# shivangchopra11/MedMoE

Measured on AMD Instinct MI355X. Metric: image-text pairs/sec at global batch 1024, higher is better.
Workload: dtype bf16; 1 GPU; cfg2: ViT-B/16 + 12-layer text tower (frozen), 8 experts top-2, 224x224x3 + 77 tokens, fwd+bwd+clip+Adam; global_batch=1024, per_gpu_batch=1024, parallelism=dp1

## Files before the change

### medmoe_amd/csrc/gemm.hip

```cpp
#include "common.h"
#include "det_plan.h"
#include <utility>

#define BM 128
#define BN 128
#define BK 64

__device__ __attribute__((aligned(256))) bf16_t g_zero_page[2048];

struct GemmNTArgs {
  const bf16_t* A; const bf16_t* B; void* C;
  const float* bias; const bf16_t* residual; bf16_t* aux;
  const int* a_rowmap; const int* c_rowmap; const int4* tiles; const int* tile_count;
  long long strideB; long long strideBias;
  int M, N, K, lda, ldb, ldc, ldr, ldaux;
  int n_tiles_n, max_tiles_m;
  float alpha; int epi; int out_f32; int col_perm;
  const int* m_dev;
};

static int g_use_nt256 = 1, g_use_nt512 = 1, g_use_tn512 = 1, g_tn_rows = 1024, g_nt_max_grid = 256, g_use_scores512 = 1, g_use_nt4w = 1, g_use_tn4w = 1, g_tn_min_rows = 2048, g_tn_rows4w = 0, g_scores_skip_epi = 0;
#ifdef NT_EXPERIMENT
__device__ int g_nt_dbg_skip = 0;
#define NT_X(...) __VA_ARGS__
#else
#define NT_X(...)
#endif
#ifdef NT_TIMING
__device__ unsigned long long g_nt_timing[8 * 8];
#define NT_T(...) __VA_ARGS__
__device__ __forceinline__ long long nt_clk() {
  __builtin_amdgcn_sched_barrier(0); const long long c = clock64(); __builtin_amdgcn_sched_barrier(0); return c;
}
#else
#define NT_T(...)
#endif
extern int g_attn_resident;
extern int g_sa_rows;
extern int g_attn_rt13;
static int g_last_nt_kernel = -1;
extern "C" int medmoe_last_gemm_nt_kernel() { return g_last_nt_kernel; }
extern int g_ln_one_row;
int g_use_nt_direct = 1;
extern "C" int medmoe_set_option(int key, int value) {
  if (key == 16) { g_ln_one_row = value; return MM_OK; }
  if (key == 17) { g_use_nt_direct = value; return MM_OK; }
  if (key == 1) { g_use_nt256 = value; return MM_OK; }
  if (key == 2) { g_use_nt512 = value; return MM_OK; }
  if (key == 3) { g_use_tn512 = value; return MM_OK; }
  if (key == 4 && value >= 256) { g_tn_rows = value; return MM_OK; }
  if (key == 5 && value >= 1 && value <= 256) { g_nt_max_grid = value; return MM_OK; }
  if (key == 6) { g_use_scores512 = value; return MM_OK; }
  if (key == 7) { g_use_nt4w = value; return MM_OK; }
  if (key == 8) { g_use_tn4w = value; return MM_OK; }
  if (key == 9 && value >= 64) { g_tn_min_rows = value; return MM_OK; }
  if (key == 12) { g_scores_skip_epi = value; return MM_OK; }
  if (key == 15 && (value == 0 || value == 448 || value == 512)) { g_attn_rt13 = value; return MM_OK; }
  if (key == 13 && value >= 0) { g_sa_rows = value; return MM_OK; }
  if (key == 11) { g_attn_resident = value; return MM_OK; }
  if (key == 10 && value >= 0) { g_tn_rows4w = value; return MM_OK; }
  return MM_ERR_ARG;
}

enum { EPI_NONE = 0, EPI_GELU = 1, EPI_RELU = 2, EPI_MUL_DGELU = 3, EPI_MUL_DRELU = 4, EPI_GELU_DAUX = 5, EPI_MUL_AUX = 6 };

struct ParkedTile {
  uint4 c[8];
  int m_base, n_base, n_items, next;
};

typedef unsigned u32x4e_t __attribute__((ext_vector_type(4)));
template <bool PARK, int TM0 = 0, int TMS = 4, int TN0 = 0, int TNS = 4, bool LDSX = false>
__device__ __forceinline__ int nt_epilogue(const GemmNTArgs& p, f32x4_t (&acc)[TMS][TNS], int m_base, int m_end,
                                           int n_base, int group, int frag_row, int frag_q, ParkedTile* park, unsigned lds_x = 0u) {
  int n_stores = 0;
  const int pg = ((frag_q & 1) << 1) | (frag_q >> 1);
  long long mc[4];
  bool mok[4];
#pragma unroll
  for (int tm = 0; tm < 4; ++tm) {
    const int m = m_base + tm * 16 + frag_row;
    mok[tm] = m < m_end;
    const int mr = min(m, m_end - 1);
    mc[tm] = p.c_rowmap ? (long long)p.c_rowmap[mr] : (long long)mr;
  }
  int nn[4];
  bool nok[4];
#pragma unroll
  for (int tn = 0; tn < 4; ++tn) {
    const int n = n_base + tn * 16 + pg * 4;
    nok[tn] = n < p.N;
    nn[tn] = min(n, p.N - 4);
  }
  float4 b4[4];
  if (p.bias) {
    const float* bias = p.bias + (long long)group * p.strideBias;
#pragma unroll
// ... 2251 lines not shown
  int u = 0;
  for (; u + 1 < U; u += 2) { substep(f0, f1); substep(f1, f0); }
  if (u < U) substep(f0, f1);
  asm volatile("s_waitcnt vmcnt(0)" ::: "memory");
  auto keep_frags = [&](Frags& f) __attribute__((always_inline)) {
#pragma unroll
    for (int ks = 0; ks < 2; ++ks) {
      asm volatile("" :: "v"(f.gl[ks][0]), "v"(f.gl[ks][1]), "v"(f.gl[ks][2]), "v"(f.gl[ks][3]), "v"(f.gh[ks][0]), "v"(f.gh[ks][1]), "v"(f.gh[ks][2]), "v"(f.gh[ks][3]));
      asm volatile("" :: "v"(f.xl[ks][0]), "v"(f.xl[ks][1]), "v"(f.xl[ks][2]), "v"(f.xl[ks][3]), "v"(f.xh[ks][0]), "v"(f.xh[ks][1]), "v"(f.xh[ks][2]), "v"(f.xh[ks][3]));
    }
  };
  if constexpr (SCALE) asm volatile("" :: "v"(wv[0][0]), "v"(wv[0][1]), "v"(wv[1][0]), "v"(wv[1][1]));
  asm volatile("s_waitcnt lgkmcnt(0)" ::: "memory");
  keep_frags(f0); keep_frags(f1);

  float* dW = p.dW + ((MAPPED || COLG) ? (long long)group * p.strideW : 0ll);
  const int kcol = lane & 31;
  const bool staged = p.partial != nullptr;
  const int pid = staged ? xcd_remap(blockIdx.x, gridDim.x) : 0;
  if (staged) {
    float* part = p.partial + ((long long)pid << 16) + (wid << 14) + lane;
#pragma unroll
    for (int tn = 0; tn < 4; ++tn)
#pragma unroll
      for (int tk = 0; tk < 4; ++tk)
#pragma unroll
        for (int r = 0; r < 16; ++r) part[((tn * 4 + tk) * 16 + r) * 64] = acc[tn][tk][r];
  } else {
#pragma unroll
  for (int tn = 0; tn < 4; ++tn)
#pragma unroll
    for (int tk = 0; tk < 4; ++tk) {
      const int k = k0 + wn * 128 + tk * 32 + kcol;
#pragma unroll
      for (int r = 0; r < 16; ++r) {
        const int n = n0 + wm * 128 + tn * 32 + (r & 3) + 8 * (r >> 2) + 4 * h;
        if ((!(MAPPED || COLG) || n < p.Nn) && (!COLG || k < p.Kk)) atomicAdd(dW + (long long)n * p.ldw + k, acc[tn][tk][r]);
      }
    }
  }
  if (do_db) {
    const bool db_staged = staged && p.db_partial != nullptr;
#pragma unroll
    for (int tn = 0; tn < 4; ++tn) {
      const float v = colsum[tn] + __shfl_xor(colsum[tn], 32, 64);
      const int n = n0 + wm * 128 + tn * 32 + kcol;
      if (db_staged) {
        if (h == 0) p.db_partial[((long long)pid << 9) + (wid << 7) + tn * 32 + kcol] = v;
      } else if (h == 0 && (!(MAPPED || COLG) || n < p.Nn)) atomicAdd(p.db + ((MAPPED || COLG) ? (long long)group * p.strideDb : 0ll) + n, v);
    }
  }
}

extern "C" int medmoe_gemm_tn(const void* G, int ldg, const void* X, int ldx, float* dW, int ldw, float* db, int M, int Nn, int Kk,
                              const int* x_rowmap, const int* g_rowmap, const int* row_off, int n_groups, long long strideW,
                              long long strideDb, int nsplit, hipStream_t stream);

__global__ __launch_bounds__(256) void tn_reduce_kernel(const float* __restrict__ partial, float* __restrict__ dW, int ldw, int ntile,
                                                        int tiles_k, int nvalid) {
  const int tile = blockIdx.x >> 6;
  const int e4 = (((blockIdx.x & 63) << 8) + threadIdx.x) << 2;
  float4 s = {0.f, 0.f, 0.f, 0.f};
  for (int sp = 0; sp < nvalid; ++sp) {
    const float4 v = *(const float4*)(partial + ((long long)(sp * ntile + tile) << 16) + e4);
    s.x += v.x; s.y += v.y; s.z += v.z; s.w += v.w;
  }
  const int lane = e4 & 63, r = (e4 >> 6) & 15, tk = (e4 >> 10) & 3, tn = (e4 >> 12) & 3, wid = e4 >> 14;
  const int wm = wid & 1, wn = wid >> 1, h = lane >> 5, kcol = lane & 31;
  const int tile_n = tile / tiles_k, tile_k = tile - tile_n * tiles_k;
  const int n = tile_n * 256 + wm * 128 + tn * 32 + (r & 3) + 8 * (r >> 2) + 4 * h;
  const int k = tile_k * 256 + wn * 128 + tk * 32 + kcol;
  float4* d = (float4*)(dW + (long long)n * ldw + k);
  float4 o = *d;
  o.x += s.x; o.y += s.y; o.z += s.z; o.w += s.w;
  *d = o;
}

struct TnReduceArgs {
  const float* partial; const float* db_partial; float* dW; float* db; const int* row_off;
  long long strideW, strideDb;
  int ldw, Nn, Kk, tiles_n, tiles_k, mode, nsplit, nvalid, n_groups, R, vec;
};
__global__ __launch_bounds__(256) void tn_reduce_det_kernel(TnReduceArgs p) {
  const int ntile = p.tiles_n * p.tiles_k;
  const int gt = blockIdx.x >> 6;
  const int group = gt / ntile, tile = gt - group * ntile;
  int first, count;
  if (p.mode == 0) { first = group * p.nsplit; count = p.nvalid; }
  else det_plan::tn_group_ranges(p.row_off, group, p.R, first, count);
  const int e4 = (((blockIdx.x & 63) << 8) + threadIdx.x) << 2;
  float4 s = {0.f, 0.f, 0.f, 0.f};
  for (int sp = 0; sp < count; ++sp) {
    const float4 v = *(const float4*)(p.partial + ((long long)((first + sp) * ntile + tile) << 16) + e4);
    s.x += v.x; s.y += v.y; s.z += v.z; s.w += v.w;
  }
  const int lane = e4 & 63, r = (e4 >> 6) & 15, tk = (e4 >> 10) & 3, tn = (e4 >> 12) & 3, wid = e4 >> 14;
  const int wm = wid & 1, wn = wid >> 1, h = lane >> 5, kcol = lane & 31;
  const int tile_n = tile / p.tiles_k, tile_k = tile - tile_n * p.tiles_k;
  const int n = tile_n * 256 + wm * 128 + tn * 32 + (r & 3) + 8 * (r >> 2) + 4 * h;
  const int k = tile_k * 256 + wn * 128 + tk * 32 + kcol;
  if (count > 0 && n < p.Nn && k < p.Kk) {
    float* d = p.dW + (long long)group * p.strideW + (long long)n * p.ldw + k;
    if (p.vec) {
      float4 o = *(float4*)d;
      o.x += s.x; o.y += s.y; o.z += s.z; o.w += s.w;
      *(float4*)d = o;
// ... 74 lines not shown
  p.gscale = nullptr; p.partial = nullptr; p.gscale_gstride = 0; p.gscale_ld = 0;
  const long long ntile = (long long)p.tiles_n * p.tiles_k * n_groups;
  p.nsplit = (int)max(1ll, min(256ll / ntile, (long long)M / g_tn_min_rows));
  if (det && p.nsplit > 1) {
    if (!scratch || ntile * p.nsplit * 65536 > scratch_floats) return MM_ERR_ARG;
    p.partial = scratch;
    const int chunk = det_plan::tn_chunk(M, p.nsplit);
    hipLaunchKernelGGL((gemm_tn4w_kernel<false, true>), dim3((unsigned)(ntile * p.nsplit)), dim3(256), 0, stream, p);
    TnReduceArgs q{scratch, nullptr, dW, nullptr, nullptr, strideW, 0, ldw, Nn, Kk, p.tiles_n, p.tiles_k, 0, p.nsplit, (M + chunk - 1) / chunk,
                   n_groups, 0, tn_vec_ok(dW, ldw, strideW) ? 1 : 0};
    hipLaunchKernelGGL(tn_reduce_det_kernel, dim3((unsigned)(ntile * 64)), dim3(256), 0, stream, q);
    return mm_check_launch();
  }
  if (p.nsplit > 1) ++g_mm_nondet;
  hipLaunchKernelGGL((gemm_tn4w_kernel<false, true>), dim3((unsigned)(ntile * p.nsplit)), dim3(256), 0, stream, p);
  return mm_check_launch();
}

extern "C" int medmoe_gemm_tn_cols(const void* G, int ldg, const void* X, int ldx, float* dW, int ldw, int M, int Nn, int Kk,
                                   int n_groups, long long gcol_stride, long long xcol_stride, long long strideW, int g_chunk_w,
                                   long long g_chunk_stride, hipStream_t stream) {
  return tn_cols_impl(G, ldg, X, ldx, dW, ldw, M, Nn, Kk, n_groups, gcol_stride, xcol_stride, strideW, g_chunk_w, g_chunk_stride, false,
                      nullptr, 0, stream);
}

extern "C" int medmoe_gemm_tn_cols_det(const void* G, int ldg, const void* X, int ldx, float* dW, int ldw, int M, int Nn, int Kk,
                                       int n_groups, long long gcol_stride, long long xcol_stride, long long strideW, int g_chunk_w,
                                       long long g_chunk_stride, float* scratch, long long scratch_floats, hipStream_t stream) {
  return tn_cols_impl(G, ldg, X, ldx, dW, ldw, M, Nn, Kk, n_groups, gcol_stride, xcol_stride, strideW, g_chunk_w, g_chunk_stride, true,
                      scratch, scratch_floats, stream);
}

extern "C" long long medmoe_gemm_tn_cols_det_scratch(int M, int Nn, int Kk, int n_groups) {
  return det_plan::cols_scratch_floats(M, Nn, Kk, n_groups, g_tn_min_rows);
}

static int tn_gram_impl(const void* A, int lda, const float* w, long long w_gstride, int w_ld, float* dW, int ldw, int M,
                        int Nn, int n_groups, long long col_stride, long long strideW, bool det, hipStream_t stream) {
  if (!A || !w || !dW) return MM_ERR_ARG;
  if (M < 32 || (M % 32) || Nn <= 0 || (Nn % 8) || (lda % 8) || n_groups < 1 || Nn > lda || w_ld < 1 || w_gstride < 0) return MM_ERR_SHAPE;
  if ((col_stride % 8) || col_stride < 0 || 32ll * lda * 2 + 1024 >= (1ll << 32) || 64ll * w_ld * 4 >= (1ll << 32)) return MM_ERR_SHAPE;
  GemmTNArgs p;
  p.partial = nullptr;
  p.G = (const bf16_t*)A; p.X = (const bf16_t*)A; p.dW = dW; p.db = nullptr;
  p.x_rowmap = nullptr; p.g_rowmap = nullptr; p.row_off = nullptr; p.strideW = strideW; p.strideDb = 0;
  p.M = M; p.Nn = Nn; p.Kk = Nn; p.ldg = lda; p.ldx = lda; p.ldw = ldw;
  p.tiles_n = (Nn + 255) / 256; p.tiles_k = p.tiles_n;
  p.n_groups = n_groups; p.gcol_stride = col_stride; p.xcol_stride = col_stride;
  p.g_chunk_w = 0; p.g_chunk_stride = 0;
  p.gscale = w; p.gscale_gstride = w_gstride; p.gscale_ld = w_ld;
  const long long ntile = (long long)p.tiles_n * p.tiles_k * n_groups;
  p.nsplit = det ? 1 : (int)max(1ll, min(256ll / ntile, (long long)M / g_tn_min_rows));
  if (p.nsplit > 1) ++g_mm_nondet;
  hipLaunchKernelGGL((gemm_tn4w_kernel<false, true, true>), dim3((unsigned)(ntile * p.nsplit)), dim3(256), 0, stream, p);
  return mm_check_launch();
}

extern "C" int medmoe_gemm_tn_gram(const void* A, int lda, const float* w, long long w_gstride, int w_ld, float* dW, int ldw, int M,
                                   int Nn, int n_groups, long long col_stride, long long strideW, hipStream_t stream) {
  return tn_gram_impl(A, lda, w, w_gstride, w_ld, dW, ldw, M, Nn, n_groups, col_stride, strideW, false, stream);
}

extern "C" int medmoe_gemm_tn_gram_det(const void* A, int lda, const float* w, long long w_gstride, int w_ld, float* dW, int ldw, int M,
                                       int Nn, int n_groups, long long col_stride, long long strideW, hipStream_t stream) {
  return tn_gram_impl(A, lda, w, w_gstride, w_ld, dW, ldw, M, Nn, n_groups, col_stride, strideW, true, stream);
}

extern "C" int medmoe_gemm_tn(const void* G, int ldg, const void* X, int ldx, float* dW, int ldw,
                              float* db, int M, int Nn, int Kk, const int* x_rowmap,
                              const int* g_rowmap, const int* row_off, int n_groups, long long strideW,
                              long long strideDb, int nsplit, hipStream_t stream) {
  if (!G || !X || !dW) return MM_ERR_ARG;
  if (M <= 0 || Nn <= 0 || Kk <= 0 || (Nn % 8) || (Kk % 8) || (ldg % 8) || (ldx % 8)) return MM_ERR_SHAPE;
  if (n_groups < 1 || nsplit < 1) return MM_ERR_ARG;
  GemmTNArgs p;
  p.partial = nullptr;
  p.G = (const bf16_t*)G; p.X = (const bf16_t*)X; p.dW = dW; p.db = db;
  p.x_rowmap = x_rowmap; p.g_rowmap = g_rowmap; p.row_off = row_off; p.strideW = strideW; p.strideDb = strideDb;
  p.M = M; p.Nn = Nn; p.Kk = Kk; p.ldg = ldg; p.ldx = ldx; p.ldw = ldw; p.gcol_stride = 0; p.xcol_stride = 0; p.g_chunk_w = 0; p.g_chunk_stride = 0; p.gscale = nullptr; p.partial = nullptr; p.gscale_gstride = 0; p.gscale_ld = 0;
  const bool fit32 = (long long)M * ldg * 2 < (1ll << 32) && (long long)M * ldx * 2 < (1ll << 32);
  if (g_use_tn512 && !x_rowmap && !g_rowmap && !row_off && n_groups == 1 && (M % 32) == 0 && (Nn % 256) == 0 && (Kk % 256) == 0 &&
      M >= 4096 && fit32) {
    p.tiles_n = Nn / 256; p.tiles_k = Kk / 256;
    const int ntile = p.tiles_n * p.tiles_k;
    p.nsplit = max(1, min(256 / ntile, M / g_tn_min_rows));
    p.n_groups = 1;
    if (p.nsplit > 1) ++g_mm_nondet;
    if (g_use_tn4w) hipLaunchKernelGGL(gemm_tn4w_kernel<false>, dim3(ntile * p.nsplit), dim3(256), 0, stream, p);
    else hipLaunchKernelGGL(gemm_tn512_kernel<false>, dim3(ntile * p.nsplit), dim3(512), 0, stream, p);
    return mm_check_launch();
  }
  if (g_use_tn512 && !(x_rowmap && g_rowmap) && (Nn % 128) == 0 && (Kk % 256) == 0 && M / n_groups >= 4096 && fit32) {
    p.tiles_n = (Nn + 255) / 256; p.tiles_k = Kk / 256;
    const int ntile = p.tiles_n * p.tiles_k;
    p.n_groups = n_groups;
    ++g_mm_nondet;
    if (g_use_tn4w && row_off) {
      long long R = g_tn_rows4w > 0 ? (g_tn_rows4w + 31) / 32 * 32 : 4096;
      p.nsplit = (int)R;
      const int max_ranges = (int)(M / R) + n_groups;
      hipLaunchKernelGGL(gemm_tn4w_kernel<true>, dim3(ntile * max_ranges), dim3(256), 0, stream, p);
      return mm_check_launch();
    }
    p.nsplit = max(1, M / n_groups / g_tn_rows);
    if (g_use_tn4w) hipLaunchKernelGGL(gemm_tn4w_kernel<true>, dim3(ntile * p.nsplit * n_groups), dim3(256), 0, stream, p);
    else hipLaunchKernelGGL(gemm_tn512_kernel<true>, dim3(ntile * p.nsplit * n_groups), dim3(512), 0, stream, p);
    return mm_check_launch();
// ... 53 lines not shown
```

### medmoe_amd/csrc/pair3.hip

```cpp
#include "common.h"

struct Pair3Args {
  const uint16_t* lp; bf16_t* dS; bf16_t* A; bf16_t* U;
  const float* lse; const bf16_t* gm; const float* wnorm; float* stats; float* d2; float* dwn;
  const int* cap_lens; const float* gsim; float* sim; float* att; const int* cap_list;
  long long row_base, ld, bstride;
  int n_cap, B, Bc, HW, HWP, T, caps_per_wg, n_chunk, pw;
  long long stat_rows;
  float temp1, temp2, eps;
};

template <int CTRL>
__device__ __forceinline__ float dpp_mov(float v) {
  return __builtin_bit_cast(float, __builtin_amdgcn_update_dpp(0, __builtin_bit_cast(int, v), CTRL, 0xf, 0xf, true));
}
__device__ __forceinline__ float row16_sum(float v) {
  v += dpp_mov<0xB1>(v);
  v += dpp_mov<0x4E>(v);
  v += dpp_mov<0x141>(v);
  v += dpp_mov<0x140>(v);
  return v;
}
#define P3_DPP4(CTRL)                                                                                          \
  "v_add_f32_dpp %0, %0, %0 " CTRL " row_mask:0xf bank_mask:0xf\n\tv_add_f32_dpp %1, %1, %1 " CTRL " row_mask:0xf bank_mask:0xf\n\t" \
  "v_add_f32_dpp %2, %2, %2 " CTRL " row_mask:0xf bank_mask:0xf\n\tv_add_f32_dpp %3, %3, %3 " CTRL " row_mask:0xf bank_mask:0xf\n\t"
__device__ __forceinline__ void row16_sum4(float& a, float& b, float& c, float& d) {
  asm volatile("s_nop 1\n\t" P3_DPP4("quad_perm:[1,0,3,2]") P3_DPP4("quad_perm:[2,3,0,1]") P3_DPP4("row_half_mirror") P3_DPP4("row_mirror")
               : "+v"(a), "+v"(b), "+v"(c), "+v"(d));
}
__device__ __forceinline__ float grp4_sum(float v) {
  v += __shfl_xor(v, 16, 64);
  v += __shfl_xor(v, 32, 64);
  return v;
}
__device__ __forceinline__ uint32_t dword_of(const uint4& v, int d) { return d == 0 ? v.x : d == 1 ? v.y : d == 2 ? v.z : v.w; }
__device__ __forceinline__ void opaque(uint4& v) { asm volatile("" : "+v"(v.x), "+v"(v.y), "+v"(v.z), "+v"(v.w)); }
__device__ __forceinline__ float bf_lo(uint32_t w) { return __uint_as_float(w << 16); }
__device__ __forceinline__ float bf_hi(uint32_t w) { return __uint_as_float(w & 0xffff0000u); }
__device__ __forceinline__ void lds_store_b32(unsigned addr, unsigned v) { asm volatile("ds_write_b32 %0, %1" :: "v"(addr), "v"(v) : "memory"); }
__device__ __forceinline__ unsigned lds_load_b32(unsigned addr) {
  unsigned v;
  asm volatile("ds_read_b32 %0, %1\n\ts_waitcnt lgkmcnt(0)" : "=v"(v) : "v"(addr) : "memory");
  return v;
}
__device__ __forceinline__ void flag_publish(unsigned addr, int epoch) {
  asm volatile("s_waitcnt lgkmcnt(0)" ::: "memory");
  lds_store_b32(addr, (unsigned)epoch);
}
__device__ __forceinline__ void flag_wait(unsigned addr, int epoch) {
  while ((int)__builtin_amdgcn_readfirstlane(lds_load_b32(addr)) < epoch) __builtin_amdgcn_s_sleep(1);
}

template <int N>
__device__ __forceinline__ void flag_wait_group(unsigned addr0, int lane, int value) {
  const unsigned addr = addr0 + min(lane, N - 1) * 4;
  while (__builtin_amdgcn_ballot_w64((int)lds_load_b32(addr) < value) != 0) __builtin_amdgcn_s_sleep(1);
}

template <int HW, int NTT, bool BWD, bool WN = false>
__global__ __launch_bounds__(1024) void local_pair3_kernel(Pair3Args p) {
  constexpr int NS = (HW + 31) / 32, HWP = ((HW + 15) / 16) * 16;
  const int pw = p.pw;
  constexpr int NRT = 2 * NS, GR = NS * 32, CPI = 16 / NTT, TP = NTT * 16;
  constexpr int NRTA = (HW - 32 * (NS - 1) > 4) ? NRT : NRT - 1;
  constexpr int OFF_L = NRT * NS * 1024, OFF_R = OFF_L + 16 * GR * 4, OFF_E = OFF_R + 2 * 16 * GR * 4, OFF_F = OFF_E + 128;
  __shared__ __attribute__((aligned(16))) char smem[OFF_F + 128];
  const int tid = threadIdx.x, lane = tid & 63, wid = __builtin_amdgcn_readfirstlane(tid >> 6);
  const int fr = lane & 15, g = lane >> 4;
  const int pid = blockIdx.x;
  const int b = pid / p.n_chunk, chunk = pid - b * p.n_chunk;
  float* Lw = (float*)(smem + OFF_L) + wid * GR;
  float* Rbase = (float*)(smem + OFF_R);
  const unsigned lds0 = (unsigned)(size_t)smem;
  const unsigned eboxA = lds0 + OFF_E, flagE = lds0 + OFF_F, flagR = flagE + 64;
  if (tid < 32) ((int*)(smem + OFF_F))[tid] = 0;
  for (int f = wid; f < NRT * NS; f += 16) {
    const int rt = f / NS, s = f - rt * NS;
    const int row = 32 * (rt >> 1) + 8 * (fr >> 2) + 4 * (rt & 1) + (fr & 3);
    *(uint4*)(smem + f * 1024 + lane * 16) = *(const uint4*)(p.gm + ((long long)b * GR + row) * GR + 32 * s + 8 * g);
  }
  __syncthreads();
  const int grp = wid / NTT, tt = wid - grp * NTT, w0 = grp * NTT;
  if (grp >= CPI) return;
  const float c1 = p.temp1 * 1.44269504088896f;
  constexpr float LN2 = 0.6931471805599453f;
  const int j_end = min(p.n_cap, (chunk + 1) * p.caps_per_wg);
  constexpr uint32_t hmin = 0xFB53u;
  const char* gfrag = smem + lane * 16;
  auto load_frags = [&](bf16x8_t (&f)[NS], int rt) __attribute__((always_inline)) {
#pragma unroll
    for (int s = 0; s < NS; ++s) f[s] = *(const bf16x8_t*)(gfrag + (rt * NS + s) * 1024);
  };
  int epoch = 0;
  for (int j = chunk * p.caps_per_wg + grp; j < j_end; j += CPI) {
    ++epoch;
    const int i = p.cap_list ? p.cap_list[j] : j;
    const int cap = max(1, min(min(p.cap_lens[i], p.T), TP));
    const int t = tt * 16 + fr;
    const float mcol = t < cap ? 1.f : 0.f;
    const float nw = p.wnorm[i * p.T + min(t, p.T - 1)];
    const float gs = (BWD && p.gsim) ? p.gsim[(long long)b * p.Bc + i] : 1.f;
    const float simv = BWD ? p.sim[(long long)b * p.Bc + i] : 0.f;
    float2 st = make_float2(0.f, 0.f);
    if (BWD) st = *(const float2*)(p.stats + ((long long)b * p.stat_rows + p.row_base + (long long)j * TP + tt * 16 + fr) * 2);
    const long long off0 = (p.row_base + (long long)j * TP + t) * p.ld + (long long)b * p.bstride + 8 * g;
    uint4 lpv[NS];
#pragma unroll
    for (int s = 0; s < NS; ++s) {
      const int h0 = 32 * s + 8 * g;
      if (32 * s + 31 < HW) lpv[s] = *(const uint4*)(p.lp + off0 + 32 * s);
      else lpv[s] = (h0 < pw) ? *(const uint4*)(p.lp + off0 + 32 * s) : make_uint4(LOGP_MIN_BITS2, LOGP_MIN_BITS2, LOGP_MIN_BITS2, LOGP_MIN_BITS2);
      if (32 * s + 31 >= HW) {
        auto fix = [&](uint32_t w, int d) -> uint32_t {
          if (h0 + 2 * d >= HW) w = (w & 0xffff0000u) | hmin;
          if (h0 + 2 * d + 1 >= HW) w = (w & 0x0000ffffu) | (hmin << 16);
          return w;
        };
        lpv[s] = make_uint4(fix(lpv[s].x, 0), fix(lpv[s].y, 1), fix(lpv[s].z, 2), fix(lpv[s].w, 3));
      }
    }
    if (lane * 4 < GR) {
      const int h0 = lane * 4;
      float4 v = make_float4(0.f, 0.f, 0.f, 0.f);
      if (h0 < HWP) v = *(const float4*)(p.lse + ((long long)b * p.Bc + i) * HWP + h0);
      if (h0 >= HW) v.x = 0.f;
      if (h0 + 1 >= HW) v.y = 0.f;
      if (h0 + 2 >= HW) v.z = 0.f;
      if (h0 + 3 >= HW) v.w = 0.f;
      *(float4*)(Lw + h0) = v;
    }
    auto lp_of = [&](int s, int e) -> float {
      const uint32_t w = dword_of(lpv[s], e >> 1);
      return h2f((uint16_t)((e & 1) ? (w >> 16) : (w & 0xffffu)));
    };
    uint4 af[NS];
    float num, n2;
    if constexpr (BWD) {
#pragma unroll
      for (int s = 0; s < NS; ++s) af[s] = (32 * s + 31 < HW || 32 * s + 8 * g < pw) ? *(const uint4*)(p.A + off0 + 32 * s) : make_uint4(0u, 0u, 0u, 0u);
    }
    auto a_of = [&](int s, int e) -> float {
      const uint32_t w = dword_of(af[s], e >> 1);
      return (e & 1) ? bf_hi(w) : bf_lo(w);
    };
    bf16x8_t fg[NS];
    auto y_tile = [&](int next) __attribute__((always_inline)) -> f32x4_t {
      f32x4_t y = {0.f, 0.f, 0.f, 0.f};
#pragma unroll
      for (int s = 0; s < NS; ++s) y = __builtin_amdgcn_mfma_f32_16x16x32_bf16(fg[s], __builtin_bit_cast(bf16x8_t, af[s]), y, 0, 0, 0);
      __builtin_amdgcn_sched_barrier(0);
      if (next >= 0) load_frags(fg, next);
      __builtin_amdgcn_sched_barrier(0);
      return y;
    };
    auto y_tile_now = [&](int rt) __attribute__((always_inline)) -> f32x4_t {
      bf16x8_t f[NS];
      load_frags(f, rt);
      f32x4_t y = {0.f, 0.f, 0.f, 0.f};
#pragma unroll
      for (int s = 0; s < NS; ++s) y = __builtin_amdgcn_mfma_f32_16x16x32_bf16(f[s], __builtin_bit_cast(bf16x8_t, af[s]), y, 0, 0, 0);
      __builtin_amdgcn_sched_barrier(0);
      return y;
    };
    if constexpr (!BWD) {
      float e1[NS][8];
      float cs = 0.f, un = 0.f;
  #pragma unroll
      for (int s = 0; s < NS; ++s) {
        const float4 La = *(const float4*)(Lw + 32 * s + 8 * g), Lb = *(const float4*)(Lw + 32 * s + 8 * g + 4);
        const float Ls[8] = {La.x, La.y, La.z, La.w, Lb.x, Lb.y, Lb.z, Lb.w};
  #pragma unroll
        for (int e = 0; e < 8; ++e) {
          const float lp = lp_of(s, e);
          const float a1 = __builtin_amdgcn_exp2f(lp);
          float x = __builtin_amdgcn_exp2f(c1 * a1);
          if (32 * s + 24 + e >= HW) x = (32 * s + 8 * g + e < HW) ? x : 0.f;
          e1[s][e] = x;
          cs += x;
          un += x * fmaf(lp, LN2, Ls[e]);
        }
        __builtin_amdgcn_sched_barrier(0);
      }
      cs = grp4_sum(cs);
      un = grp4_sum(un);
      const float cinv = mcol / fmaxf(cs, 1e-30f);
      num = un * cinv;
  #pragma unroll
      for (int s = 0; s < NS; ++s) {
        float a[8];
  #pragma unroll
        for (int e = 0; e < 8; ++e) a[e] = e1[s][e] * cinv;
        const uint4 av = make_uint4(pack2bf(a[0], a[1]), pack2bf(a[2], a[3]), pack2bf(a[4], a[5]), pack2bf(a[6], a[7]));
        af[s] = av;
        if (32 * s + 31 < HW || 32 * s + 8 * g < pw) *(uint4*)(p.A + off0 + 32 * s) = av;
      }
      __builtin_amdgcn_sched_barrier(0);
  #pragma unroll
      for (int s = 0; s < NS; ++s) { opaque(lpv[s]); opaque(af[s]); }
      load_frags(fg, 0);
      n2 = 0.f;
  #pragma unroll
      for (int rt = 0; rt < NRTA; ++rt) {
        const f32x4_t y = y_tile(rt + 1 < NRTA ? rt + 1 : -1);
  #pragma unroll
        for (int r = 0; r < 4; ++r) n2 += a_of(rt >> 1, 4 * (rt & 1) + r) * y[r];
        __builtin_amdgcn_sched_barrier(0);
      }
      n2 = grp4_sum(n2);
      if (g == 0) *(float2*)(p.stats + ((long long)b * p.stat_rows + p.row_base + (long long)j * TP + t) * 2) = make_float2(num, n2);
    } else {
      num = st.x; n2 = st.y;
    }
    const float n2c = fmaxf(n2, 0.f);
    const float den = nw * sqrtf(n2c);
    const float cosv = num / fmaxf(den, p.eps);
    const float ev = (t < cap) ? __expf(p.temp2 * cosv) : 0.f;
    float se;
    if constexpr (!BWD) {
      se = row16_sum(ev);
      if (NTT > 1) {
        const unsigned eb = eboxA + (epoch & 1) * 64;
        lds_store_b32(eb + wid * 4, __float_as_uint(se));
        flag_publish(flagE + wid * 4, epoch);
        se = 0.f;
#pragma unroll
        for (int q = 0; q < NTT; ++q) {
          flag_wait(flagE + (w0 + q) * 4, epoch);
          se += __uint_as_float(lds_load_b32(eb + (w0 + q) * 4));
        }
      }
    } else se = __expf(simv);
    if (!BWD) {
      if (tt == 0 && lane == 0) p.sim[(long long)b * p.Bc + i] = __logf(se);
      if (p.att && b == i && t < p.T) {
#pragma unroll
        for (int s = 0; s < NS; ++s)
#pragma unroll
          for (int e = 0; e < 8; ++e) {
            const int hw = 32 * s + 8 * g + e;
            if (hw < HW) p.att[((long long)i * p.T + t) * HW + hw] = a_of(s, e);
          }
      }
      continue;
    }
    float dn = 0.f, d2 = 0.f;
    {
      const float dcos = gs * p.temp2 * ev / se;
      if (den >= p.eps) { dn = dcos / den; d2 = -dcos * cosv / fmaxf(n2c, 1e-30f); }
      else dn = dcos / p.eps;
      if (WN && g == 0)
        p.dwn[(long long)b * p.stat_rows + p.row_base + (long long)j * TP + t] = (den >= p.eps) ? -dcos * cosv / (nw * nw) : 0.f;
    }
    const float ca = dn * num + d2 * n2;
    const float k1 = p.temp1 * dn, k2 = p.temp1 * d2, k3 = p.temp1 * ca;
#pragma unroll
    for (int s = 0; s < NS; ++s) { opaque(lpv[s]); opaque(af[s]); }
    if (p.d2 && g == 0) p.d2[(long long)b * p.stat_rows + p.row_base + (long long)j * TP + t] = d2;

    if (p.U) {
#pragma unroll
      for (int s = 0; s < NS; ++s) {
        if (32 * s + 31 < HW || 32 * s + 8 * g < pw) {
          float u[8];
#pragma unroll
          for (int e = 0; e < 8; ++e) u[e] = a_of(s, e) * d2;
          *(uint4*)(p.U + off0 + 32 * s) = make_uint4(pack2bf(u[0], u[1]), pack2bf(u[2], u[3]), pack2bf(u[4], u[5]), pack2bf(u[6], u[7]));
        }
      }
    }
    __builtin_amdgcn_sched_barrier(0);
    float* Rall = Rbase + (epoch & 1) * 16 * GR;
    float* Rw = Rall + wid * GR;
    const int fl0 = epoch * 8 + 1;
    auto finish_block = [&](int sp, const float (&da)[8]) __attribute__((always_inline)) {
      flag_wait_group<NTT>(flagR + w0 * 4, lane, fl0 + sp);
      float ds[8];
#pragma unroll
      for (int h = 0; h < 2; ++h) {
        if (2 * sp + h < NRTA) {
          float rd[4] = {0.f, 0.f, 0.f, 0.f};
#pragma unroll
          for (int q = 0; q < NTT; ++q) {
            const float4 v = *(const float4*)(Rall + (w0 + q) * GR + 32 * sp + 8 * g + 4 * h);
            rd[0] += v.x; rd[1] += v.y; rd[2] += v.z; rd[3] += v.w;
          }
#pragma unroll
          for (int r = 0; r < 4; ++r) {
            const float a1 = __builtin_amdgcn_exp2f(lp_of(sp, 4 * h + r));
            const float a = a_of(sp, 4 * h + r);
            ds[4 * h + r] = dn * a + a1 * (da[4 * h + r] - rd[r]);
          }
        } else {
#pragma unroll
          for (int r = 0; r < 4; ++r) ds[4 * h + r] = 0.f;
        }
        __builtin_amdgcn_sched_barrier(0);
      }
      if (32 * sp + 31 < HW || 32 * sp + 8 * g < pw)
        *(uint4*)(p.dS + off0 + 32 * sp) = make_uint4(pack2bf(ds[0], ds[1]), pack2bf(ds[2], ds[3]), pack2bf(ds[4], ds[5]), pack2bf(ds[6], ds[7]));
      __builtin_amdgcn_sched_barrier(0);
    };
#pragma unroll
    for (int s = 0; s < NS; ++s) { opaque(lpv[s]); opaque(af[s]); }
    float dap[8];
#pragma unroll
    for (int sp = 0; sp < NS; ++sp) {
      float dac[8], ds[8];
#pragma unroll
      for (int h = 0; h < 2; ++h) {
        const int rt = 2 * sp + h;
        if (rt < NRTA) {
          const float4 L4 = *(const float4*)(Lw + 32 * sp + 8 * g + 4 * h);
          const f32x4_t y = y_tile_now(rt);
          const float Lr[4] = {L4.x, L4.y, L4.z, L4.w};
          float pr[4], a1[4];
#pragma unroll
          for (int r = 0; r < 4; ++r) {
            const float lp = lp_of(sp, 4 * h + r);
            a1[r] = __builtin_amdgcn_exp2f(lp);
            const float a = a_of(sp, 4 * h + r);
            const float da1 = a * (k1 * fmaf(lp, LN2, Lr[r]) + (k2 * y[r] - k3));
            dac[4 * h + r] = da1;
            pr[r] = a1[r] * da1;
          }
          row16_sum4(pr[0], pr[1], pr[2], pr[3]);
          if (NTT > 1) {
            if (fr == 0) *(float4*)(Rw + 32 * sp + 8 * g + 4 * h) = make_float4(pr[0], pr[1], pr[2], pr[3]);
          } else {
#pragma unroll
            for (int r = 0; r < 4; ++r) ds[4 * h + r] = dn * a_of(sp, 4 * h + r) + a1[r] * (dac[4 * h + r] - pr[r]);
          }
        } else {
#pragma unroll
          for (int r = 0; r < 4; ++r) { dac[4 * h + r] = 0.f; ds[4 * h + r] = 0.f; }
        }
        __builtin_amdgcn_sched_barrier(0);
      }
      if (NTT > 1) {
        flag_publish(flagR + wid * 4, fl0 + sp);
        if (sp > 0) {
          opaque(lpv[sp - 1]); opaque(af[sp - 1]);
          finish_block(sp - 1, dap);
        }
#pragma unroll
        for (int e = 0; e < 8; ++e) dap[e] = dac[e];
      } else if (32 * sp + 31 < HW || 32 * sp + 8 * g < pw)
        *(uint4*)(p.dS + off0 + 32 * sp) = make_uint4(pack2bf(ds[0], ds[1]), pack2bf(ds[2], ds[3]), pack2bf(ds[4], ds[5]), pack2bf(ds[6], ds[7]));
    }
    if (NTT > 1) {
      opaque(lpv[NS - 1]); opaque(af[NS - 1]);
      finish_block(NS - 1, dap);
    }
  }
}

static int g_pair3_chunks = 0;
extern "C" int medmoe_local_pair3_chunks(int n) {
  if (n < 0) return MM_ERR_ARG;
  g_pair3_chunks = n;
  return MM_OK;
}

extern "C" int medmoe_local_pair3_supported(int HW, int T) {
  const int ntt = (T + 15) / 16;
  return ((HW == 64 && ntt == 1) || (HW == 196 && ntt >= 1 && ntt <= 5)) ? 1 : 0;
}

static int pair3_launch(const void* lp, void* dS, void* A, void* U, const float* lse, const void* gm, const float* wnorm,
                        const int* cap_lens, const float* gsim, float* sim, float* att, float* stats, long long stat_rows,
                        int B, int Bc, int HW, int T, float temp1, float temp2, float eps, const int* cap_list, int n_cap,
                        int ntt, long long row_base, long long ld, long long bstride, int pw, float* d2, float* dwn, hipStream_t stream);

extern "C" int medmoe_local_pair3(const void* lp, void* dS, void* A, void* U, const float* lse, const void* gm, const float* wnorm,
                                  const int* cap_lens, const float* gsim, float* sim, float* att, float* stats, long long stat_rows,
                                  int B, int Bc, int HW, int T, float temp1, float temp2, float eps, const int* cap_list, int n_cap,
                                  int ntt, long long row_base, long long ld, long long bstride, int pw, float* d2, hipStream_t stream) {
  return pair3_launch(lp, dS, A, U, lse, gm, wnorm, cap_lens, gsim, sim, att, stats, stat_rows, B, Bc, HW, T, temp1, temp2, eps, cap_list, n_cap, ntt,
                      row_base, ld, bstride, pw, d2, nullptr, stream);
}

extern "C" int medmoe_local_pair3_wgrad(const void* lp, void* dS, void* A, void* U, const float* lse, const void* gm, const float* wnorm,
                                        const int* cap_lens, const float* gsim, float* sim, float* att, float* stats, long long stat_rows,
                                        int B, int Bc, int HW, int T, float temp1, float temp2, float eps, const int* cap_list, int n_cap,
                                        int ntt, long long row_base, long long ld, long long bstride, int pw, float* d2, float* dwn,
                                        hipStream_t stream) {
  if (!dS || !dwn) return MM_ERR_ARG;
  return pair3_launch(lp, dS, A, U, lse, gm, wnorm, cap_lens, gsim, sim, att, stats, stat_rows, B, Bc, HW, T, temp1, temp2, eps, cap_list, n_cap, ntt,
                      row_base, ld, bstride, pw, d2, dwn, stream);
}

static int pair3_launch(const void* lp, void* dS, void* A, void* U, const float* lse, const void* gm, const float* wnorm,
                        const int* cap_lens, const float* gsim, float* sim, float* att, float* stats, long long stat_rows,
                        int B, int Bc, int HW, int T, float temp1, float temp2, float eps, const int* cap_list, int n_cap,
                        int ntt, long long row_base, long long ld, long long bstride, int pw, float* d2, float* dwn, hipStream_t stream) {
  if (dS && !U && !d2) return MM_ERR_ARG;
  if (!lp || !lse || !gm || !wnorm || !cap_lens || !A || !sim || !stats) return MM_ERR_ARG;
  if (stat_rows < row_base + (long long)n_cap * ntt * 16) return MM_ERR_SHAPE;
  if (B <= 0 || Bc <= 0 || n_cap <= 0 || (ld % 8) || (bstride % 8) || (pw % 8) || pw < HW || pw > ((HW + 31) / 32) * 32 || ntt < 1 || ntt > 5 || ntt * 16 > ((T + 15) / 16) * 16) return MM_ERR_SHAPE;
  if (!medmoe_local_pair3_supported(HW, ntt * 16)) return MM_ERR_SHAPE;
  Pair3Args p;
  p.lp = (const uint16_t*)lp; p.dS = (bf16_t*)dS; p.A = (bf16_t*)A; p.U = (bf16_t*)U;
  p.lse = lse; p.gm = (const bf16_t*)gm; p.wnorm = wnorm; p.stats = stats; p.d2 = d2; p.dwn = dwn; p.stat_rows = stat_rows; p.cap_lens = cap_lens; p.gsim = gsim; p.sim = sim; p.att = att;
  p.cap_list = cap_list; p.row_base = row_base; p.ld = ld; p.bstride = bstride; p.n_cap = n_cap; p.B = B; p.Bc = Bc; p.HW = HW;
  p.HWP = ((HW + 15) / 16) * 16; p.pw = pw; p.T = T; p.temp1 = temp1; p.temp2 = temp2; p.eps = eps;
  const int cpi = 16 / ntt;
  int n_chunk = g_pair3_chunks > 0 ? g_pair3_chunks : max(1, (1024 + B - 1) / B);
  int cpw = ((n_cap + n_chunk - 1) / n_chunk + cpi - 1) / cpi * cpi;
  n_chunk = (n_cap + cpw - 1) / cpw;
  p.caps_per_wg = cpw; p.n_chunk = n_chunk;
  const dim3 grid(B * n_chunk), block(1024);
#define P3(HW_, T_)                                                                                       \
  { if (dS && dwn) hipLaunchKernelGGL((local_pair3_kernel<HW_, T_, true, true>), grid, block, 0, stream, p);   \
    else if (dS) hipLaunchKernelGGL((local_pair3_kernel<HW_, T_, true>), grid, block, 0, stream, p);           \
    else hipLaunchKernelGGL((local_pair3_kernel<HW_, T_, false>), grid, block, 0, stream, p); }
  if (HW == 64) P3(64, 1)
  else switch (ntt) { case 1: P3(196, 1) break; case 2: P3(196, 2) break; case 3: P3(196, 3) break; case 4: P3(196, 4) break; default: P3(196, 5) break; }
#undef P3
  return mm_check_launch();
}
```

Measured before the change: 4789 pairs/s.

## Add specialized 224-wide gram TN kernel and streamline pair3 loads

```diff
diff --git a/medmoe_amd/csrc/gemm.hip b/medmoe_amd/csrc/gemm.hip
--- a/medmoe_amd/csrc/gemm.hip
+++ b/medmoe_amd/csrc/gemm.hip
@@ -42,7 +42,11 @@
 extern "C" int medmoe_last_gemm_nt_kernel() { return g_last_nt_kernel; }
 extern int g_ln_one_row;
 int g_use_nt_direct = 1;
+static int g_use_gram7 = 1;
+extern int g_pair3_pad_loads;
 extern "C" int medmoe_set_option(int key, int value) {
+  if (key == 18) { g_use_gram7 = value; return MM_OK; }
+  if (key == 19) { g_pair3_pad_loads = value; return MM_OK; }
   if (key == 16) { g_ln_one_row = value; return MM_OK; }
   if (key == 17) { g_use_nt_direct = value; return MM_OK; }
   if (key == 1) { g_use_nt256 = value; return MM_OK; }
@@ -2400,6 +2404,202 @@
   }
 }
 
+__global__ __launch_bounds__(256) void gemm_tn_gram7_kernel(GemmTNArgs p) {
+  __shared__ __attribute__((aligned(128))) char smem[4 * SUB3 + 4096];
+  const int tid = threadIdx.x, lane = tid & 63, wid = __builtin_amdgcn_readfirstlane(tid >> 6);
+  const int id = xcd_remap(blockIdx.x, gridDim.x);
+  const int group = id / p.nsplit, split = id - group * p.nsplit;
+  int ms, me;
+  det_plan::tn_split_range(p.M, p.nsplit, split, ms, me);
+  if (ms >= me) return;
+  const int U = (me - ms + 31) / 32;
+
+  const int prow = (wid << 1) + (lane >> 5);
+  const unsigned lds0 = (unsigned)(size_t)smem;
+  unsigned col_g, col_x;
+  {
+    const int lc0 = (lane & 31) ^ ((prow & 3) << 2);
+    const int col = lc0 * 8;
+    col_g = (unsigned)(col >= p.Nn ? 0 : col) * 2u;
+    col_x = (unsigned)(col >= p.Kk ? 0 : col) * 2u;
+  }
+  const unsigned ldg2 = (unsigned)p.ldg * 2u, ldx2 = (unsigned)p.ldx * 2u;
+  int lk = 0, wb = 0, rb = 0;
+  unsigned sg[4], sx[4];
+  const char* gbase = (const char*)p.G + (long long)group * p.gcol_stride * 2;
+  const char* xbase = (const char*)p.X + (long long)group * p.xcol_stride * 2;
+  const char* gsub = gbase;
+  const char* xsub = xbase;
+  const char* wbase = (const char*)(p.gscale + (long long)group * p.gscale_gstride);
+  const char* wsub = wbase;
+  int wr0 = 0;
+  const unsigned wl0 = lds0 + 4 * SUB3 + wid * 1024;
+  auto setup_rows = [&]() __attribute__((always_inline)) {
+    const long long r0 = ms + min(lk, (me - ms) / 32 - 1) * 32;
+    auto uni = [](const char* q) -> const char* {
+      const unsigned long long v = (unsigned long long)q;
+      const unsigned lo = __builtin_amdgcn_readfirstlane((unsigned)v), hi = __builtin_amdgcn_readfirstlane((unsigned)(v >> 32));
+      return (const char*)(((unsigned long long)hi << 32) | lo);
+    };
+    gsub = uni(gbase + r0 * (long long)ldg2);
+    xsub = uni(xbase + r0 * (long long)ldx2);
+    wr0 = (int)r0; wsub = uni(wbase + r0 * (long long)p.gscale_ld * 4);
+  };
+#pragma unroll
+  for (int j = 0; j < 4; ++j) { sg[j] = (unsigned)(prow + 8 * j) * ldg2 + col_g; sx[j] = (unsigned)(prow + 8 * j) * ldx2 + col_x; }
+  unsigned ldsW = lds0 + wid * 1024;
+  auto advance = [&]() __attribute__((always_inline)) {
+    ++lk; wb = (wb + 1) & 3;
+    setup_rows();
+    ldsW = lds0 + wb * SUB3 + wid * 1024;
+  };
+  auto piece = [&](int i) __attribute__((always_inline)) {
+    __builtin_amdgcn_global_load_lds(GLB_PTR((i < 4 ? gsub : xsub) + (i < 4 ? sg[i & 3] : sx[i & 3])),
+                                     (__attribute__((address_space(3))) void*)(size_t)(ldsW + i * 4096), 16, 0, 0);
+  };
+  auto wpiece = [&]() __attribute__((always_inline)) {
+    const unsigned wo = (unsigned)min(lane, p.M - 1 - wr0) * (unsigned)p.gscale_ld * 4u;
+    __builtin_amdgcn_global_load_lds(GLB_PTR(wsub + wo), (__attribute__((address_space(3))) void*)(size_t)(wl0 + wb * 256), 4, 0, 0);
+  };
+
+  f32x16_t acc[2][7];
+#pragma unroll
+  for (int i = 0; i < 2; ++i)
+#pragma unroll
+    for (int j = 0; j < 7; ++j)
+#pragma unroll
+      for (int r = 0; r < 16; ++r) acc[i][j][r] = 0.f;
+
+  const int h = lane >> 5, gam = (lane >> 4) & 1, q = (lane & 15) >> 2, pp = lane & 3;
+  unsigned aa[9];
+#pragma unroll
+  for (int t = 0; t < 9; ++t) {
+    const int c = (t < 2 ? (2 * wid + t) * 4 : (t - 2) * 4) + gam * 2 + (pp >> 1);
+    aa[t] = lds0 + (t < 2 ? 0 : 16384) + (8 * h + q) * 512 + ((c ^ (q << 2)) << 4) + ((pp & 1) << 3);
+  }
+  struct Frags { u32x2_t gl[2][2], gh[2][2], xl[2][7], xh[2][7]; };
+  Frags f0, f1;
+  u32x4_t wv[2][2];
+  const unsigned wa = wl0 + 32 * (lane >> 5);
+  auto read_w = [&](int buf) __attribute__((always_inline)) {
+    const unsigned a = wa + buf * 256;
+    W_READ(wv[0][0], a, 0); W_READ(wv[0][1], a, 16); W_READ(wv[1][0], a, 64); W_READ(wv[1][1], a, 80);
+  };
+  auto scale_frag = [&](Frags& f, auto ksc, auto tnc) __attribute__((always_inline)) {
+    constexpr int ks = decltype(ksc)::value, tn = decltype(tnc)::value;
+    auto sc = [](unsigned v, unsigned w0, unsigned w1) -> unsigned {
+      return pack2bf(__uint_as_float(v << 16) * __uint_as_float(w0), __uint_as_float(v & 0xffff0000u) * __uint_as_float(w1));
+    };
+    const u32x4_t wl = wv[ks][0], wh = wv[ks][1];
+    f.gl[ks][tn][0] = sc(f.gl[ks][tn][0], wl[0], wl[1]); f.gl[ks][tn][1] = sc(f.gl[ks][tn][1], wl[2], wl[3]);
+    f.gh[ks][tn][0] = sc(f.gh[ks][tn][0], wh[0], wh[1]); f.gh[ks][tn][1] = sc(f.gh[ks][tn][1], wh[2], wh[3]);
+  };
+  auto read_one = [&](Frags& f, unsigned bo, auto gc) __attribute__((always_inline)) {
+    constexpr int g = decltype(gc)::value, gx = g < 8 ? g : g - 8, t = gx >> 2, ks = (gx >> 1) & 1, hi = gx & 1;
+    constexpr int off = ks * 8192 + hi * 2048;
+    const unsigned a = aa[g < 8 ? t : 2 + t] + bo;
+    if constexpr (g < 8) { if constexpr (hi) TR_READ(f.gh[ks][t], a, off); else TR_READ(f.gl[ks][t], a, off); }
+    else { if constexpr (hi) TR_READ(f.xh[ks][t], a, off); else TR_READ(f.xl[ks][t], a, off); }
+  };
+  auto frag = [&](u32x2_t lo, u32x2_t hi) -> bf16x8_t {
+    const uint4 v = make_uint4(lo[0], lo[1], hi[0], hi[1]);
+    return __builtin_bit_cast(bf16x8_t, v);
+  };
+  const bool two = wid < 3;
+  auto substep = [&](Frags& c, Frags& n) __attribute__((always_inline)) {
+    constexpr int NT = 2, NM = 14 * NT, W = NM - 4, NR = 36, RLO = NR / W, RNH = NR - RLO * W;
+    const unsigned bo = rb * SUB3;
+    auto one = [&](auto qc) __attribute__((always_inline)) {
+      constexpr int qq = decltype(qc)::value, fi = qq / 7, ks = fi / NT, tn = fi % NT, tk = qq % 7;
+      if (tn == 0 || two)
+        acc[tn][tk] = __builtin_amdgcn_mfma_f32_32x32x16_bf16(frag(c.gl[ks][tn], c.gh[ks][tn]), frag(c.xl[ks][tk], c.xh[ks][tk]), acc[tn][tk], 0, 0, 0);
+      if constexpr (qq < W) {
+        __builtin_amdgcn_sched_barrier(0);
+        constexpr int r0 = qq < RNH ? qq * (RLO + 1) : RNH * (RLO + 1) + (qq - RNH) * RLO, r1 = r0 + (qq < RNH ? RLO + 1 : RLO);
+        auto rd = [&](auto jc) __attribute__((always_inline)) { read_one(n, bo, std::integral_constant<int, r0 + decltype(jc)::value>{}); };
+        static_for<r1 - r0>(rd);
+        auto pc = [&](auto jc) __attribute__((always_inline)) {
+          constexpr int j = decltype(jc)::value;
+          if constexpr ((j * W) / 8 == qq) piece(j);
+        };
+        static_for<8>(pc);
+        if constexpr (qq == 0) wpiece();
+        if constexpr (tk == 0 && fi + 1 < 2 * NT)
+          scale_frag(c, std::integral_constant<int, (fi + 1) / NT>{}, std::integral_constant<int, (fi + 1) % NT>{});
+        if constexpr (qq == 7 * (2 * NT - 2)) read_w(rb);
+        if constexpr (qq == W - 1) { advance(); rb = (rb + 1) & 3; }
+        __builtin_amdgcn_sched_barrier(0);
+      }
+      if constexpr (qq == W - 1) {
+        __builtin_amdgcn_sched_barrier(0);
+        asm volatile("s_waitcnt lgkmcnt(0)\n\ts_waitcnt vmcnt(16)" ::: "memory");
+        __builtin_amdgcn_s_barrier();
+        __builtin_amdgcn_sched_barrier(0);
+        asm volatile("" ::: "memory");
+      }
+      if constexpr (qq == W) {
+        __builtin_amdgcn_sched_barrier(0);
+        scale_frag(n, std::integral_constant<int, 0>{}, std::integral_constant<int, 0>{});
+        __builtin_amdgcn_sched_barrier(0);
+      }
+    };
+    static_for<NM>(one);
+  };
+
+  setup_rows();
+  for (int v = 0; v < 4; ++v) {
+    wpiece();
+#pragma unroll
+    for (int i = 0; i < 8; ++i) piece(i);
+    advance();
+  }
+  asm volatile("s_waitcnt vmcnt(24)" ::: "memory");
+  __builtin_amdgcn_s_barrier();
+  asm volatile("" ::: "memory");
+  {
+    auto rd = [&](auto gc) __attribute__((always_inline)) { read_one(f0, 0u, gc); };
+    static_for<36>(rd);
+    read_w(0);
+  }
+  rb = 1;
+  asm volatile("s_waitcnt lgkmcnt(0)\n\ts_waitcnt vmcnt(16)" ::: "memory");
+  __builtin_amdgcn_s_barrier();
+  __builtin_amdgcn_sched_barrier(0);
+  asm volatile("" ::: "memory");
+  scale_frag(f0, std::integral_constant<int, 0>{}, std::integral_constant<int, 0>{});
+  int u = 0;
+  for (; u + 1 < U; u += 2) { substep(f0, f1); substep(f1, f0); }
+  if (u < U) substep(f0, f1);
+  asm volatile("s_waitcnt vmcnt(0)" ::: "memory");
+  auto keep_frags = [&](Frags& f) __attribute__((always_inline)) {
+#pragma unroll
+    for (int ks = 0; ks < 2; ++ks) {
+      asm volatile("" :: "v"(f.gl[ks][0]), "v"(f.gl[ks][1]), "v"(f.gh[ks][0]), "v"(f.gh[ks][1]));
+      asm volatile("" :: "v"(f.xl[ks][0]), "v"(f.xl[ks][1]), "v"(f.xl[ks][2]), "v"(f.xl[ks][3]), "v"(f.xl[ks][4]), "v"(f.xl[ks][5]), "v"(f.xl[ks][6]));
+      asm volatile("" :: "v"(f.xh[ks][0]), "v"(f.xh[ks][1]), "v"(f.xh[ks][2]), "v"(f.xh[ks][3]), "v"(f.xh[ks][4]), "v"(f.xh[ks][5]), "v"(f.xh[ks][6]));
+    }
+  };
+  asm volatile("" :: "v"(wv[0][0]), "v"(wv[0][1]), "v"(wv[1][0]), "v"(wv[1][1]));
+  asm volatile("s_waitcnt lgkmcnt(0)" ::: "memory");
+  keep_frags(f0); keep_frags(f1);
+
+  float* dW = p.dW + (long long)group * p.strideW;
+  const int kcol = lane & 31;
+#pragma unroll
+  for (int tn = 0; tn < 2; ++tn) {
+    if (tn == 1 && !two) break;
+#pragma unroll
+    for (int tk = 0; tk < 7; ++tk) {
+      const int k = tk * 32 + kcol;
+#pragma unroll
+      for (int r = 0; r < 16; ++r) {
+        const int n = (2 * wid + tn) * 32 + (r & 3) + 8 * (r >> 2) + 4 * h;
+        if (n < p.Nn && k < p.Kk) atomicAdd(dW + (long long)n * p.ldw + k, acc[tn][tk][r]);
+      }
+    }
+  }
+}
+
 extern "C" int medmoe_gemm_tn(const void* G, int ldg, const void* X, int ldx, float* dW, int ldw, float* db, int M, int Nn, int Kk,
                               const int* x_rowmap, const int* g_rowmap, const int* row_off, int n_groups, long long strideW,
                               long long strideDb, int nsplit, hipStream_t stream);
@@ -2580,7 +2780,8 @@
   const long long ntile = (long long)p.tiles_n * p.tiles_k * n_groups;
   p.nsplit = det ? 1 : (int)max(1ll, min(256ll / ntile, (long long)M / g_tn_min_rows));
   if (p.nsplit > 1) ++g_mm_nondet;
-  hipLaunchKernelGGL((gemm_tn4w_kernel<false, true, true>), dim3((unsigned)(ntile * p.nsplit)), dim3(256), 0, stream, p);
+  if (g_use_gram7 && Nn > 192 && Nn <= 224) hipLaunchKernelGGL(gemm_tn_gram7_kernel, dim3((unsigned)(ntile * p.nsplit)), dim3(256), 0, stream, p);
+  else hipLaunchKernelGGL((gemm_tn4w_kernel<false, true, true>), dim3((unsigned)(ntile * p.nsplit)), dim3(256), 0, stream, p);
   return mm_check_launch();
 }
 
diff --git a/medmoe_amd/csrc/pair3.hip b/medmoe_amd/csrc/pair3.hip
--- a/medmoe_amd/csrc/pair3.hip
+++ b/medmoe_amd/csrc/pair3.hip
@@ -5,6 +5,7 @@
   const float* lse; const bf16_t* gm; const float* wnorm; float* stats; float* d2; float* dwn;
   const int* cap_lens; const float* gsim; float* sim; float* att; const int* cap_list;
   long long row_base, ld, bstride;
+  int pad_loads;
   int n_cap, B, Bc, HW, HWP, T, caps_per_wg, n_chunk, pw;
   long long stat_rows;
   float temp1, temp2, eps;
@@ -92,24 +93,56 @@
     for (int s = 0; s < NS; ++s) f[s] = *(const bf16x8_t*)(gfrag + (rt * NS + s) * 1024);
   };
   int epoch = 0;
+  int i_nx = 0, len_nx = 1;
+  auto fetch_cap = [&](int jj) __attribute__((always_inline)) {
+    const int jc = min(jj, p.n_cap - 1);
+    i_nx = p.cap_list ? p.cap_list[jc] : jc; len_nx = p.cap_lens[i_nx];
+  };
+  fetch_cap(chunk * p.caps_per_wg + grp);
   for (int j = chunk * p.caps_per_wg + grp; j < j_end; j += CPI) {
     ++epoch;
-    const int i = p.cap_list ? p.cap_list[j] : j;
-    const int cap = max(1, min(min(p.cap_lens[i], p.T), TP));
+    const int i = i_nx;
+    const int cap = max(1, min(min(len_nx, p.T), TP));
+    fetch_cap(j + CPI);
     const int t = tt * 16 + fr;
     const float mcol = t < cap ? 1.f : 0.f;
+    const bool ldrow = t < cap || p.pad_loads;
+    auto uni = [](const void* q) -> char* {
+      const unsigned long long v = (unsigned long long)q;
+      const unsigned lo = __builtin_amdgcn_readfirstlane((unsigned)v), hi = __builtin_amdgcn_readfirstlane((unsigned)(v >> 32));
+      return (char*)(((unsigned long long)hi << 32) | lo);
+    };
+    const long long wrow = (long long)b * p.stat_rows + p.row_base + (long long)j * TP + tt * 16;
     const float nw = p.wnorm[i * p.T + min(t, p.T - 1)];
     const float gs = (BWD && p.gsim) ? p.gsim[(long long)b * p.Bc + i] : 1.f;
     const float simv = BWD ? p.sim[(long long)b * p.Bc + i] : 0.f;
     float2 st = make_float2(0.f, 0.f);
-    if (BWD) st = *(const float2*)(p.stats + ((long long)b * p.stat_rows + p.row_base + (long long)j * TP + tt * 16 + fr) * 2);
-    const long long off0 = (p.row_base + (long long)j * TP + t) * p.ld + (long long)b * p.bstride + 8 * g;
-    uint4 lpv[NS];
+    if (BWD) st = *(const float2*)(uni(p.stats + wrow * 2) + (unsigned)fr * 8u);
+    const long long ubase = ((p.row_base + (long long)j * TP + tt * 16) * p.ld + (long long)b * p.bstride) * 2;
+    const unsigned voff = ((unsigned)fr * (unsigned)p.ld + 8u * (unsigned)g) * 2u;
+    const char* lpb = uni((const char*)p.lp + ubase);
+    char* Ab = uni((char*)p.A + ubase);
+    char* Ub = uni((char*)p.U + ubase);
+    char* dSb = uni((char*)p.dS + ubase);
+    uint4 lpv[NS], af[NS];
+#pragma unroll
+    for (int s = 0; s < NS; ++s) {
+      lpv[s] = make_uint4(LOGP_MIN_BITS2, LOGP_MIN_BITS2, LOGP_MIN_BITS2, LOGP_MIN_BITS2);
+      if (BWD) af[s] = make_uint4(0u, 0u, 0u, 0u);
+    }
+    if (ldrow) {
+#pragma unroll
+      for (int s = 0; s < NS; ++s)
+        if (32 * s + 31 < HW || 32 * s + 8 * g < pw) lpv[s] = *(const uint4*)(lpb + voff + 64 * s);
+      if constexpr (BWD) {
+#pragma unroll
+        for (int s = 0; s < NS; ++s)
+          if (32 * s + 31 < HW || 32 * s + 8 * g < pw) af[s] = *(const uint4*)(Ab + voff + 64 * s);
+      }
+    }
 #pragma unroll
     for (int s = 0; s < NS; ++s) {
       const int h0 = 32 * s + 8 * g;
-      if (32 * s + 31 < HW) lpv[s] = *(const uint4*)(p.lp + off0 + 32 * s);
-      else lpv[s] = (h0 < pw) ? *(const uint4*)(p.lp + off0 + 32 * s) : make_uint4(LOGP_MIN_BITS2, LOGP_MIN_BITS2, LOGP_MIN_BITS2, LOGP_MIN_BITS2);
       if (32 * s + 31 >= HW) {
         auto fix = [&](uint32_t w, int d) -> uint32_t {
           if (h0 + 2 * d >= HW) w = (w & 0xffff0000u) | hmin;
@@ -122,7 +155,7 @@
     if (lane * 4 < GR) {
       const int h0 = lane * 4;
       float4 v = make_float4(0.f, 0.f, 0.f, 0.f);
-      if (h0 < HWP) v = *(const float4*)(p.lse + ((long long)b * p.Bc + i) * HWP + h0);
+      if (h0 < HWP) v = *(const float4*)(uni(p.lse + ((long long)b * p.Bc + i) * HWP) + (unsigned)lane * 16u);
       if (h0 >= HW) v.x = 0.f;
       if (h0 + 1 >= HW) v.y = 0.f;
       if (h0 + 2 >= HW) v.z = 0.f;
@@ -133,12 +166,7 @@
       const uint32_t w = dword_of(lpv[s], e >> 1);
       return h2f((uint16_t)((e & 1) ? (w >> 16) : (w & 0xffffu)));
     };
-    uint4 af[NS];
     float num, n2;
-    if constexpr (BWD) {
-#pragma unroll
-      for (int s = 0; s < NS; ++s) af[s] = (32 * s + 31 < HW || 32 * s + 8 * g < pw) ? *(const uint4*)(p.A + off0 + 32 * s) : make_uint4(0u, 0u, 0u, 0u);
-    }
     auto a_of = [&](int s, int e) -> float {
       const uint32_t w = dword_of(af[s], e >> 1);
       return (e & 1) ? bf_hi(w) : bf_lo(w);
@@ -192,7 +220,7 @@
         for (int e = 0; e < 8; ++e) a[e] = e1[s][e] * cinv;
         const uint4 av = make_uint4(pack2bf(a[0], a[1]), pack2bf(a[2], a[3]), pack2bf(a[4], a[5]), pack2bf(a[6], a[7]));
         af[s] = av;
-        if (32 * s + 31 < HW || 32 * s + 8 * g < pw) *(uint4*)(p.A + off0 + 32 * s) = av;
+        if (32 * s + 31 < HW || 32 * s + 8 * g < pw) *(uint4*)(Ab + voff + 64 * s) = av;
       }
       __builtin_amdgcn_sched_barrier(0);
   #pragma unroll
@@ -207,7 +235,7 @@
         __builtin_amdgcn_sched_barrier(0);
       }
       n2 = grp4_sum(n2);
-      if (g == 0) *(float2*)(p.stats + ((long long)b * p.stat_rows + p.row_base + (long long)j * TP + t) * 2) = make_float2(num, n2);
+      if (g == 0) *(float2*)(uni(p.stats + wrow * 2) + (unsigned)fr * 8u) = make_float2(num, n2);
     } else {
       num = st.x; n2 = st.y;
     }
@@ -249,13 +277,13 @@
       if (den >= p.eps) { dn = dcos / den; d2 = -dcos * cosv / fmaxf(n2c, 1e-30f); }
       else dn = dcos / p.eps;
       if (WN && g == 0)
-        p.dwn[(long long)b * p.stat_rows + p.row_base + (long long)j * TP + t] = (den >= p.eps) ? -dcos * cosv / (nw * nw) : 0.f;
+        *(float*)(uni(p.dwn + wrow) + (unsigned)fr * 4u) = (den >= p.eps) ? -dcos * cosv / (nw * nw) : 0.f;
     }
     const float ca = dn * num + d2 * n2;
     const float k1 = p.temp1 * dn, k2 = p.temp1 * d2, k3 = p.temp1 * ca;
 #pragma unroll
     for (int s = 0; s < NS; ++s) { opaque(lpv[s]); opaque(af[s]); }
-    if (p.d2 && g == 0) p.d2[(long long)b * p.stat_rows + p.row_base + (long long)j * TP + t] = d2;
+    if (p.d2 && g == 0) *(float*)(uni(p.d2 + wrow) + (unsigned)fr * 4u) = d2;
 
     if (p.U) {
 #pragma unroll
@@ -264,7 +292,7 @@
           float u[8];
 #pragma unroll
           for (int e = 0; e < 8; ++e) u[e] = a_of(s, e) * d2;
-          *(uint4*)(p.U + off0 + 32 * s) = make_uint4(pack2bf(u[0], u[1]), pack2bf(u[2], u[3]), pack2bf(u[4], u[5]), pack2bf(u[6], u[7]));
+          *(uint4*)(Ub + voff + 64 * s) = make_uint4(pack2bf(u[0], u[1]), pack2bf(u[2], u[3]), pack2bf(u[4], u[5]), pack2bf(u[6], u[7]));
         }
       }
     }
@@ -297,7 +325,7 @@
         __builtin_amdgcn_sched_barrier(0);
       }
       if (32 * sp + 31 < HW || 32 * sp + 8 * g < pw)
-        *(uint4*)(p.dS + off0 + 32 * sp) = make_uint4(pack2bf(ds[0], ds[1]), pack2bf(ds[2], ds[3]), pack2bf(ds[4], ds[5]), pack2bf(ds[6], ds[7]));
+        *(uint4*)(dSb + voff + 64 * sp) = make_uint4(pack2bf(ds[0], ds[1]), pack2bf(ds[2], ds[3]), pack2bf(ds[4], ds[5]), pack2bf(ds[6], ds[7]));
       __builtin_amdgcn_sched_barrier(0);
     };
 #pragma unroll
@@ -345,7 +373,7 @@
 #pragma unroll
         for (int e = 0; e < 8; ++e) dap[e] = dac[e];
       } else if (32 * sp + 31 < HW || 32 * sp + 8 * g < pw)
-        *(uint4*)(p.dS + off0 + 32 * sp) = make_uint4(pack2bf(ds[0], ds[1]), pack2bf(ds[2], ds[3]), pack2bf(ds[4], ds[5]), pack2bf(ds[6], ds[7]));
+        *(uint4*)(dSb + voff + 64 * sp) = make_uint4(pack2bf(ds[0], ds[1]), pack2bf(ds[2], ds[3]), pack2bf(ds[4], ds[5]), pack2bf(ds[6], ds[7]));
     }
     if (NTT > 1) {
       opaque(lpv[NS - 1]); opaque(af[NS - 1]);
@@ -355,6 +383,7 @@
 }
 
 static int g_pair3_chunks = 0;
+int g_pair3_pad_loads = 0;
 extern "C" int medmoe_local_pair3_chunks(int n) {
   if (n < 0) return MM_ERR_ARG;
   g_pair3_chunks = n;
@@ -398,11 +427,12 @@
   if (stat_rows < row_base + (long long)n_cap * ntt * 16) return MM_ERR_SHAPE;
   if (B <= 0 || Bc <= 0 || n_cap <= 0 || (ld % 8) || (bstride % 8) || (pw % 8) || pw < HW || pw > ((HW + 31) / 32) * 32 || ntt < 1 || ntt > 5 || ntt * 16 > ((T + 15) / 16) * 16) return MM_ERR_SHAPE;
   if (!medmoe_local_pair3_supported(HW, ntt * 16)) return MM_ERR_SHAPE;
+  if (ld <= 0 || ld >= (1ll << 27)) return MM_ERR_SHAPE;
   Pair3Args p;
   p.lp = (const uint16_t*)lp; p.dS = (bf16_t*)dS; p.A = (bf16_t*)A; p.U = (bf16_t*)U;
   p.lse = lse; p.gm = (const bf16_t*)gm; p.wnorm = wnorm; p.stats = stats; p.d2 = d2; p.dwn = dwn; p.stat_rows = stat_rows; p.cap_lens = cap_lens; p.gsim = gsim; p.sim = sim; p.att = att;
   p.cap_list = cap_list; p.row_base = row_base; p.ld = ld; p.bstride = bstride; p.n_cap = n_cap; p.B = B; p.Bc = Bc; p.HW = HW;
-  p.HWP = ((HW + 15) / 16) * 16; p.pw = pw; p.T = T; p.temp1 = temp1; p.temp2 = temp2; p.eps = eps;
+  p.HWP = ((HW + 15) / 16) * 16; p.pad_loads = g_pair3_pad_loads; p.pw = pw; p.T = T; p.temp1 = temp1; p.temp2 = temp2; p.eps = eps;
   const int cpi = 16 / ntt;
   int n_chunk = g_pair3_chunks > 0 ? g_pair3_chunks : max(1, (1024 + B - 1) / B);
   int cpw = ((n_cap + n_chunk - 1) / n_chunk + cpi - 1) / cpi * cpi;
```

Result: no change. 4815 pairs/s, median of 6 (+0.5%).
